# Tomeu7/AO-MARL

Measured on AMD Instinct MI355X. Metric: env steps/sec (AO frames/sec), higher is better.
Workload: dtype f32

## Files before the change

ao_marl_amd/csrc/aomarl_capi.hip:

```cpp
#include "aomarl_kernels.hip"

#include <math.h>
#include <stdlib.h>
#include <stdarg.h>
#include <stdio.h>
#include <string.h>

#include <algorithm>
#include <climits>
#include <string>
#include <vector>

static thread_local char g_err[512] = "";

int fail(const char *fmt, ...) {
  va_list ap;
  va_start(ap, fmt);
  vsnprintf(g_err, sizeof(g_err), fmt, ap);
  va_end(ap);
  return 1;
}


struct aomarl_ctx {
// ... 49 lines not shown
  bool frame_marked = false;
  struct FramePipe {
    bool have_twin = false, active = false;
    const float *owner_screens = nullptr;
    aomarl_state twin;
    int par = 0;
    hipStream_t fstream = nullptr;
    hipEvent_t ev_cmd = nullptr, ev_commit = nullptr, ev_done[2] = {nullptr, nullptr}, ev_psf[2] = {nullptr, nullptr};
    hipEvent_t ev_done_cur[2] = {nullptr, nullptr};
    bool psf_out[2] = {false, false};
    bool cmd_covers_commit = false;
    bool cmd_covers_psf = false;
    int32_t *snap[2] = {nullptr, nullptr};
    size_t snap_ints = 0;
    unsigned long long steps = 0, overlapped = 0, behind = 0;
  } pipe;
  int32_t *snap_target = nullptr;
  bool snap_complete = false;
  bool pipe_enabled = true;
  bool pipe_internal = false;
  hipEvent_t ev_frame_prev = nullptr;
  bool need_prev = false, group_overlap = false;
  bool psf_side = false;
  const float *pre_screens = nullptr;
  int pre_b = 0, pre_n = 0;
  float *cmat = nullptr;
  int ld_cmat = 0;
  int nmodes = 0, nact = 0, ld_v2m = 0, ld_m2v = 0;
  float *v2m = nullptr, *m2v = nullptr, *freedom = nullptr;
  float *s2m = nullptr;
  int s2m_nmodes = 0;
// ... 78 lines not shown

static bool is_int(float v) { return floorf(v) == v; }

int aomarl_create(const aomarl_desc *d, aomarl_ctx **out) {
  if (!d || !out) return fail("aomarl_create: null argument");
  if (d->abi_version != AOMARL_ABI_VERSION)
    return fail("aomarl_create: ABI version %d, library is %d", d->abi_version, AOMARL_ABI_VERSION);
  if (d->nlayers < 0 || d->nlayers > AOMARL_MAX_LAYERS) return fail("nlayers out of range");
  if (d->ndm < 1 || d->ndm > AOMARL_MAX_DMS) return fail("ndm out of range");
  if (d->n <= 0 || d->pupdiam <= 0 || d->n < d->pupdiam) return fail("bad pupil sizes");
  if (d->pupdiam % 4 || d->n % 4) return fail("pupil grid sizes must be multiples of 4");
  if (d->npsf & (d->npsf - 1)) return fail("npsf must be a power of two");
  if (!(d->strehl_halfwin == 4 || d->strehl_halfwin == 8 || d->strehl_halfwin == 16))
    return fail("strehl_halfwin must be 4, 8 or 16");
  aomarl_ctx *c = new aomarl_ctx();
  DevSys &s = c->sys;
  memset(&s, 0, sizeof(s));
  int rc = 0;
#define UP(T, host, n, dev)                                      \
  do {                                                           \
    T *_p;                                                       \
    rc = upload<T>(c, host, n, &_p);                             \
    if (rc) { aomarl_destroy(c); return rc; }                    \
    dev = _p;                                                    \
  } while (0)
  s.n = d->n; s.pupdiam = d->pupdiam;
  UP(float, d->mpupil, (size_t)d->n * d->n, s.mpupil);
  UP(float, d->spupil, (size_t)d->pupdiam * d->pupdiam, s.spupil);
  c->h_spupil.assign(d->spupil, d->spupil + (size_t)d->pupdiam * d->pupdiam);
  s.nvalid = d->nvalid; s.pdiam = d->pdiam; s.nfft = d->nfft; s.npix = d->npix;
// ... 397 lines not shown
  if (!c) return 0;
  for (void *p : c->owned) (void)hipFree(p);
  for (int k = 0; k < 2; k++) {
    if (c->pipe.snap[k]) (void)hipFree(c->pipe.snap[k]);
    if (c->pipe.ev_done[k]) (void)hipEventDestroy(c->pipe.ev_done[k]);
    if (c->pipe.ev_psf[k]) (void)hipEventDestroy(c->pipe.ev_psf[k]);
  }
  if (c->ev_reset) (void)hipEventDestroy(c->ev_reset);
  for (int k = 0; k < 3; k++) if (c->ev_reset2[k]) (void)hipEventDestroy(c->ev_reset2[k]);
  if (c->pipe.ev_cmd) (void)hipEventDestroy(c->pipe.ev_cmd);
  if (c->pipe.ev_commit) (void)hipEventDestroy(c->pipe.ev_commit);
  if (c->pipe.fstream) { (void)hipStreamSynchronize(c->pipe.fstream); (void)hipStreamDestroy(c->pipe.fstream); }
  if (c->atm_stream) (void)hipStreamSynchronize(c->atm_stream);
  if (c->psf_stream) (void)hipStreamSynchronize(c->psf_stream);
  if (c->ev_frame) (void)hipEventDestroy(c->ev_frame);
  if (c->ev_moved) (void)hipEventDestroy(c->ev_moved);
  if (c->ev_psf) (void)hipEventDestroy(c->ev_psf);
  if (c->env_gain) (void)hipFree(c->env_gain);
  if (c->seed_stage) (void)hipFree(c->seed_stage);
  rp_free(c);
  if (c->timg) (void)hipFree(c->timg);
  for (hipEvent_t e : c->fw_ev) (void)hipEventDestroy(e);
  for (hipEvent_t e : c->fw_ev_retired) (void)hipEventDestroy(e);
  delete c;
  return 0;
}

static int replace_dev(aomarl_ctx *c, float **slot, const std::vector<float> &h) {
  if (*slot) {
    for (size_t i = 0; i < c->owned.size(); i++)
      if (c->owned[i] == *slot) { c->owned.erase(c->owned.begin() + i); break; }
// ... 186 lines not shown
```

ao_marl_amd/csrc/aomarl_capi_atmos.hip:

```cpp
static int side_stream(aomarl_ctx *c) {
  if (!c->atm_stream) {
    int prio_lo = 0, prio_hi = 0;
    HIPCHK(hipDeviceGetStreamPriorityRange(&prio_lo, &prio_hi));
    static hipStream_t g_atm[64] = {nullptr}, g_psf[64] = {nullptr};
    int dev = 0;
    HIPCHK(hipGetDevice(&dev));
    if (dev < 0 || dev >= 64) return fail("side_stream: device ordinal %d", dev);
    if (!g_atm[dev]) {
      HIPCHK(hipStreamCreateWithPriority(&g_atm[dev], hipStreamNonBlocking, 0));
      HIPCHK(hipStreamCreateWithPriority(&g_psf[dev], hipStreamNonBlocking, prio_lo));
    }
    c->atm_stream = g_atm[dev]; c->psf_stream = g_psf[dev];
    HIPCHK(hipEventCreateWithFlags(&c->ev_frame, hipEventDisableTiming));
    c->ev_frame_cur = c->ev_frame;
    HIPCHK(hipEventCreateWithFlags(&c->ev_moved, hipEventDisableTiming));
    HIPCHK(hipEventCreateWithFlags(&c->ev_psf, hipEventDisableTiming));
    HIPCHK(hipEventCreateWithFlags(&c->ev_fork, hipEventDisableTiming));
  }
  return 0;
}
static int psf_wait_pending(aomarl_ctx *c, void *stream) {
  if (c->psf_side && !c->side_joined) HIPCHK(hipStreamWaitEvent((hipStream_t)stream, c->ev_psf, 0));
  c->psf_side = false;
  return 0;
// ... 128 lines not shown
    for (int j = 0; j < i; j++)
      if (layer[j] == layer[i]) return fail("extrude: a layer appears twice in one round");
    ops.layer[i] = layer[i]; ops.dir[i] = dir[i]; ops.tflag[i] = 0;
  }
  return extrude_rounds(c, st, b, n, &ops, 1, stream);
}

struct Plan { int kx[AOMARL_MAX_LAYERS], ky[AOMARL_MAX_LAYERS]; };

static bool plan_eq(const Plan &a, const Plan &b, int nl) {
  for (int l = 0; l < nl; l++)
    if (a.kx[l] != b.kx[l] || a.ky[l] != b.ky[l]) return false;
  return true;
}

static int run_plan(aomarl_ctx *c, aomarl_state *st, int b, int n, const Plan &p, void *stream) {
  int maxr = 0;
  for (int l = 0; l < c->nlayers; l++) {
    int len = abs(p.kx[l]) + abs(p.ky[l]);
    if (len > maxr) maxr = len;
  }
  for (int l = 0; l < c->nlayers; l++)
    if (p.kx[l] == 0 && p.ky[l] == 0) c->snap_complete = false;
  if (maxr == 0) return 0;
  if ((hipStream_t)stream != c->atm_stream || !c->atm_stream) { int rc = atmos_wait_pending(c, stream); if (rc) return rc; }
  c->group_overlap = false;
  if (c->ev_frame_prev) {
    bool fits = true;
    for (int l = 0; l < c->nlayers; l++) {
      const DevLayer &L = c->sys.layers[l];
// ... 511 lines not shown
```

ao_marl_amd/csrc/aomarl_capi_stages.hip:

```cpp
static int dm_shape_impl(aomarl_ctx *c, aomarl_state *st, int b, int n, const float *volts,
                         bool skip_stack, void *stream) {
  const float *v = volts ? volts : st->voltage + (size_t)b * st->ld_actu;
  const int ldv = volts ? c->sys.nactu : st->ld_actu;
  DevState ds = dev_state(st);
  for (int k = 0; k < c->ndm; k++) {
    const DevDm &D = c->sys.dms[k];
    const int np = D.dim * D.dim;
    if (D.type == AOMARL_DM_TT)
      hipLaunchKernelGGL(k_dm_shape, dim3(1, n), dim3(64), 0, (hipStream_t)stream, c->sys, ds, b, k, v, ldv);
    else if (skip_stack)
      continue;
    else if (D.sep && !c->force_generic_dm)
      hipLaunchKernelGGL(k_dm_shape_sep, dim3((D.dim + DMS_TX - 1) / DMS_TX, (D.dim + DMS_TY - 1) / DMS_TY, n),
                         dim3(256), 0, (hipStream_t)stream, c->sys, ds, b, k, v, ldv);
    else
      hipLaunchKernelGGL(k_dm_shape, dim3((np + 255) / 256, n), dim3(256), 0, (hipStream_t)stream, c->sys, ds, b, k, v, ldv);
    LAUNCHCHK();
  }
  return 0;
}

int aomarl_comp_dm_shape(aomarl_ctx *c, aomarl_state *st, int b, int n, const float *volts, void *stream) {
  int rc = check_range(c, st, b, n);
  if (rc) return rc;
// ... 24 lines not shown
    g_gemm_kgroups = value;
    return 0;
  }
  if (!strcmp(name, "gemm_xcd_map")) { g_gemm_xcd = value != 0; return 0; }
  if (!strcmp(name, "gemm_target_blocks")) { g_gemm_target_blocks = value > 0 ? value : 0; return 0; }
  if (!strcmp(name, "gemm_split_f16")) { g_gemm_split_f16 = value != 0; return 0; }
  if (!strcmp(name, "precision")) return aomarl_set_precision(value);
  if (!c) return fail("set_option: null context");
  if (!strcmp(name, "force_generic_dm")) { c->force_generic_dm = value != 0; return 0; }
  if (!strcmp(name, "force_valu_target")) { c->force_valu_target = value != 0; return 0; }
  if (!strcmp(name, "defer_dm_shape")) { c->defer_dm_shape = value != 0; return 0; }
  if (!strcmp(name, "frame_pipeline")) {
    if (c->pipe.active) return fail("frame_pipeline: a frame is in flight (reset first)");
    c->pipe_enabled = value != 0; return 0;
  }
  if (!strcmp(name, "small_move")) { c->small_move = value != 0; return 0; }
  if (!strcmp(name, "small_chain")) { c->small_chain = value != 0; return 0; }
  if (!strcmp(name, "renew_frame_stream")) {
    auto &P = c->pipe;
    if (P.active) return fail("renew_frame_stream: a frame is in flight (reset first)");
    if (P.fstream) {
      HIPCHK(hipStreamSynchronize(P.fstream));
      HIPCHK(hipStreamDestroy(P.fstream));
      P.fstream = nullptr;
      HIPCHK(hipStreamCreateWithFlags(&P.fstream, hipStreamNonBlocking));
    }
    return 0;
  }
  if (!strcmp(name, "residual_shortcut")) {
    if (value && (!c->s2m || c->s2m_nmodes < 1)) return fail("residual_shortcut: no v2m . cmat matrix (aomarl_set_slopes2modes)");
// ... 394 lines not shown
```

ao_marl_amd/csrc/aomarl_capi_step.hip:

```cpp
long long aomarl_actor_tiled_floats(int n_agents, int N, int K) {
  return (long long)n_agents * ((N + 15) / 16) * ((K + 15) / 16) * 256;
}

int aomarl_actor_tile_weights(int n_agents, int N, int K, const float *src, float *dst, void *stream) {
  if (!src || !dst) return fail("actor_tile_weights: null pointer");
  if (n_agents <= 0 || N <= 0 || K <= 0) return fail("actor_tile_weights: bad sizes");
  const int ntile = (N + 15) / 16, ksteps = (K + 15) / 16;
  const long long per = (long long)ntile * ksteps * 256;
  hipLaunchKernelGGL(k_actor_tile_weights, dim3((unsigned)((per + 255) / 256), n_agents), dim3(256), 0,
                     (hipStream_t)stream, N, K, ntile, ksteps, src, dst);
  LAUNCHCHK();
  return 0;
}

int aomarl_actor_forward(const aomarl_actor_desc *d, const float *state, const float *eps, uint32_t seed,
                         uint32_t counter, float *action, float *mean, void *stream) {
  if (!d || !state || !action || !mean) return fail("actor_forward: null argument");
  if (d->n_hidden < 1 || d->n_hidden > 8) return fail("actor_forward: 1..8 hidden layers");
  const int A = d->n_agents, n = d->nenv, H = d->hidden;
  if (A <= 0 || n <= 0) return 0;
  if (!(d->flags & AOMARL_ACTOR_LAYER_BY_LAYER) && d->W1_tiled && d->Whead_tiled && H % 16 == 0) {
    const int ks1 = (d->in_max + 15) / 16, nto = (2 * d->act_max + 15) / 16;
    const size_t img1 = (size_t)256 * std::max(H / 16, nto), img0 = std::max((size_t)256 * ks1, img1);
    const size_t lds = (img0 + img1 + d->act_max + 4) * sizeof(float);
// ... 96 lines not shown
      if (k < K) a0 = fmaf(xs[k], row[k], a0);
    }
    float y = a0 + a1;
    y += __shfl_xor(y, 1);
    y += __shfl_xor(y, 2);
    if (o < no && q == 0) done(o, y);
  }
}
struct SmallHead {
  int nm, na, nact, n_agents, ld_m2v, ld_actu, ktt, do_strehl;
  float gain, factor, wa, wb, wc;
  const float *m0, *m1, *action, *freedom, *m2v, *PEND;
  const int32_t *amode_inv, *lohi;
  float *modes_out, *rew;
};
__global__ __launch_bounds__(256) void k_small_head(DevSys sys, DevState st, SmallHead p) {
  __shared__ float sm[SMALL_NM], sv[SMALL_NA];
  const int e = blockIdx.x, tid = threadIdx.x, lane = tid & 63, wv = tid >> 6;
  for (int m = tid; m < p.nm; m += 256) {
    float v = p.m0[(long long)e * p.nm + m] + p.gain * p.m1[(long long)e * p.nm + m];
    if (p.action) {
      const int j = p.amode_inv[m];
      if (j >= 0) v += p.action[(long long)e * p.nact + j] * p.freedom[m];
    }
    sm[m] = v;
    if (p.modes_out) p.modes_out[(long long)e * p.nm + m] = v;
  }
  if (p.rew)
    for (int a = wv; a < p.n_agents; a += 4) {
      const int lo = p.lohi[2 * a], hi = p.lohi[2 * a + 1];
      float q = 0.f;
      for (int m = lo + lane; m < hi; m += 64) { const float v = p.m1[(long long)e * p.nm + m]; q += v * v; }
      q = wave_sum(q);
// ... 67 lines not shown
  return c->small_chain && c->sys.nactu <= SMALL_NA && c->sys.nslope <= SMALL_NSL && g->nmodes <= SMALL_NM &&
         (long long)c->sys.nactu * c->sys.nslope <= 65536 && c->cmat && !c->env_gain;
}

static bool env_step_fusable(aomarl_ctx *c, const aomarl_env_glue *g, int *ktt_out) {
  int ktt = -1, ntt = 0, nother = 0;
  for (int k = 0; k < c->ndm; k++) {
    if (c->sys.dms[k].type == AOMARL_DM_TT) { ktt = k; ntt++; } else nother++;
  }
  const bool defer = c->defer_dm_shape && aomarl_dm_from_voltage_available(c);
  if (ktt_out) *ktt_out = ktt;
  return !(g->flags & AOMARL_ENV_STEP_UNFUSED) && ntt == 1 && (defer || nother == 0);
}

static int env_step_head_fused(aomarl_ctx *c, aomarl_state *st, aomarl_state *stv, aomarl_env_glue *g, const float *action,
                               float gain, float *reward_out, int ktt, bool ahead, hipEvent_t psf_ev, void *stream) {
  hipStream_t s = (hipStream_t)stream;
  const int n = st->nenv, nm = g->nmodes, R = g->nhist + 1, na = c->sys.nactu;
  const size_t slot = (size_t)n * nm;
  float *newest = g->modes_ring + (size_t)g->ring_pos * slot;
  float *mnew = g->modes_ring + (size_t)((g->ring_pos + 1) % R) * slot;
  Work w = work_layout(c, st->nenv);
  DevState dsv = dev_state(stv);
  if (small_chain_ok(c, g)) {
    const float d = c->delay;
    SmallHead p;
    if (d <= 1.f) { p.wa = 1.f - d; p.wb = d; p.wc = 0.f; } else { p.wa = 0.f; p.wb = 2.f - d; p.wc = d - 1.f; }
    if (ahead) { p.wa = p.wb; p.wb = p.wc; p.wc = 0.f; }
    p.nm = nm; p.na = na; p.nact = c->nact; p.n_agents = reward_out ? g->n_agents : 0; p.ld_m2v = c->ld_m2v;
    p.ld_actu = st->ld_actu; p.ktt = ktt; p.do_strehl = 1; p.gain = gain; p.factor = g->reward_factor;
    p.m0 = newest; p.m1 = g->res_modes; p.action = action; p.freedom = c->freedom; p.m2v = c->m2v;
    p.PEND = stv->work + w.PEND; p.amode_inv = c->amode_inv; p.lohi = g->lohi; p.modes_out = mnew; p.rew = reward_out;
    if (psf_ev) HIPCHK(hipStreamWaitEvent(s, psf_ev, 0));
    else if (stv == st) { int rc = psf_wait_pending(c, stream); if (rc) return rc; }
    hipExtLaunchKernelGGL(k_small_head, dim3(n), dim3(256), 0, s, nullptr, ahead ? c->pipe.ev_cmd : nullptr, 0, c->sys, dsv, p);
    LAUNCHCHK();
    if (ahead) c->pipe.cmd_covers_commit = true;
    return 0;
  }
  float *modes = st->work + w.MODES;
  const int cx = (nm + 255) / 256;
  bool psf_waited = false;
  if (ahead && psf_ev) { HIPCHK(hipStreamWaitEvent(s, psf_ev, 0)); psf_waited = true; }
  hipLaunchKernelGGL(k_compose_rewards, dim3(cx + (reward_out ? g->n_agents : 0), n), dim3(256), 0, s, nm, newest,
                     g->res_modes, gain, action, c->nact, c->amode_inv, c->freedom, modes, w.ldm, mnew, cx,
                     g->n_agents, g->lohi, g->reward_factor, reward_out);
  LAUNCHCHK();
  int nsp = 0;
  float alpha = 1.f;
  launch_gemm_nt(n, na, nm, 1.0f, modes, w.ldm, c->m2v, c->ld_m2v, 0.0f, st->com, st->ld_actu, s,
                 st->work + w.GEMM, w.gemm_floats, nullptr, &nsp, true, 16.f, c->m2v_scale, &alpha, 288);
  LAUNCHCHK();
  const float d = c->delay;
  float wa, wb, wc;
  if (d <= 1.f) { wa = 1.f - d; wb = d; wc = 0.f; } else { wa = 0.f; wb = 2.f - d; wc = d - 1.f; }
  if (ahead) {
    hipExtLaunchKernelGGL(k_delay_ahead, dim3((na + 255) / 256, 2 * n), dim3(256), 0, s, nullptr, c->pipe.ev_cmd, 0, c->sys, dsv, na,
                          st->ld_actu, n, nsp > 0 ? st->work + w.GEMM : nullptr, nsp, alpha, ktt);
    LAUNCHCHK();
    c->pipe.cmd_covers_psf = psf_waited;
  } else {
    if (nsp > 0)
      hipLaunchKernelGGL(k_delay_sum, dim3((na + 255) / 256, n), dim3(256), 0, s, dsv, na, st->ld_actu, wa, wb, wc, 0, 1,
                         st->work + w.GEMM, nsp, alpha, n);
    else
      hipLaunchKernelGGL(k_delay, dim3((na + 255) / 256, n), dim3(256), 0, s, dsv, na, st->ld_actu, wa, wb, wc, 0, 1);
    LAUNCHCHK();
  }
  if (psf_ev) { if (!psf_waited) HIPCHK(hipStreamWaitEvent(s, psf_ev, 0)); }
  else if (stv == st) { int rc = psf_wait_pending(c, stream); if (rc) return rc; }
  hipLaunchKernelGGL(k_post_delay, dim3(ahead ? n : 2 * n), dim3(256), 0, s, c->sys, dsv, 0, n, stv->work + w.PEND, 1, ktt,
                     stv->voltage, st->ld_actu);
  LAUNCHCHK();
// ... 154 lines not shown
  const auto &P = c->pipe;
  return P.have_twin && c->pipe_enabled && P.owner_screens == st->screens && !c->graph_step && !c->capturing && c->prefetch_atmos &&
         c->delay == 1.f && c->sys.noise < 0.f && !g->denoiser && accumx && accumy && !c->subpixel_flow &&
         aomarl_frame_fused_available(c) && c->defer_dm_shape && aomarl_dm_from_voltage_available(c) &&
         env_step_fusable(c, g, nullptr);
}

static int pipe_init(aomarl_ctx *c, const aomarl_state *st) {
  auto &P = c->pipe;
  int rc = side_stream(c);
  if (rc) return rc;
  if (!P.fstream) {
    HIPCHK(hipStreamCreateWithFlags(&P.fstream, hipStreamNonBlocking));
    HIPCHK(hipEventCreateWithFlags(&P.ev_cmd, hipEventDisableTiming));
    HIPCHK(hipEventCreateWithFlags(&P.ev_commit, hipEventDisableTiming));
    for (int k = 0; k < 2; k++) {
      HIPCHK(hipEventCreateWithFlags(&P.ev_done[k], hipEventDisableTiming));
      HIPCHK(hipEventCreateWithFlags(&P.ev_psf[k], hipEventDisableTiming));
    }
  }
  const size_t ints = (size_t)st->nenv * c->nlayers * 2;
  if (P.snap_ints < ints) {
    for (int k = 0; k < 2; k++) {
      if (P.snap[k]) (void)hipFree(P.snap[k]);
      P.snap[k] = nullptr;
      HIPCHK(hipMalloc((void **)&P.snap[k], sizeof(int32_t) * ints));
    }
    P.snap_ints = ints;
  }
  return 0;
}

static int pipe_launch_frame(aomarl_ctx *c, aomarl_state *st, int q, void *stream) {
  auto &P = c->pipe;
  (void)stream;
  HIPCHK(hipStreamWaitEvent(P.fstream, P.ev_cmd, 0));
  if (!c->premoved || c->pre_screens != st->screens || c->pre_b != 0 || c->pre_n != st->nenv)
    return fail("frame pipeline: no prefetched atmosphere frame of the whole batch is pending");
  HIPCHK(hipStreamWaitEvent(P.fstream, c->ev_moved, 0));
  c->premoved = false;
  aomarl_state v = pipe_view(c, st, q);
  v.origin = P.snap[q];
  return frame_fused_impl(c, &v, 0, st->nenv, AOMARL_IMG_COG | AOMARL_IMG_NOISE | AOMARL_IMG_DM_FROM_VOLTAGE,
                          (void *)P.fstream, q);
}

static int pipe_prefetch(aomarl_ctx *c, aomarl_state *st, float *accumx, float *accumy, int older, int newest) {
  auto &P = c->pipe;
  if (c->premoved) return fail("frame pipeline: a prefetched frame is already pending");
  c->side_joined = false;
  c->ev_frame_prev = P.ev_done_cur[older]; c->need_prev = true;
  c->ev_frame_cur = P.ev_done_cur[newest]; c->frame_wait_pending = true;
  c->snap_target = P.snap[older]; c->snap_complete = true;
  c->ride_ev = c->ev_moved; c->rode = false;
  int rc = move_atmos_now(c, st, 0, st->nenv, accumx, accumy, (void *)c->atm_stream);
  c->ride_ev = nullptr;
  const bool complete = c->snap_complete;
  c->snap_target = nullptr;
  if (!rc && !complete && c->need_prev && c->frame_wait_pending)
    rc = hipStreamWaitEvent(c->atm_stream, c->ev_frame_prev, 0) == hipSuccess ? 0 : fail("frame pipeline: hipStreamWaitEvent failed");
  c->ev_frame_prev = nullptr; c->need_prev = false; c->frame_wait_pending = false; c->group_overlap = false;
  if (rc) return rc;
  if (!complete)
    HIPCHK(hipMemcpyAsync(P.snap[older], st->origin, sizeof(int32_t) * (size_t)st->nenv * c->nlayers * 2,
                          hipMemcpyDeviceToDevice, c->atm_stream));
  c->screens_dirty_main = false;
  if (!(c->rode && complete)) HIPCHK(hipEventRecord(c->ev_moved, c->atm_stream));
  c->premoved = true; c->pre_screens = st->screens; c->pre_b = 0; c->pre_n = st->nenv;
  return 0;
}

static int env_step_pipelined(aomarl_ctx *c, aomarl_state *st, aomarl_env_glue *g, const float *action, float gain,
                              float *accumx, float *accumy, float *state_out, float *reward_out, void *stream) {
// ... 12 lines not shown
    HIPCHK(hipEventRecord(P.ev_psf[0], c->psf_stream));
    P.psf_out[0] = true; P.psf_out[1] = false;
    c->psf_side = false;
    aomarl_state v1 = pipe_view(c, st, 1);
    HIPCHK(hipMemcpyAsync(v1.voltage, st->com1, sizeof(float) * (size_t)n * st->ld_actu, hipMemcpyDeviceToDevice, s));
    Work w = work_layout(c, st->nenv);
    hipLaunchKernelGGL(k_post_delay, dim3(2 * n), dim3(256), 0, s, c->sys, dev_state(&v1), 0, n, v1.work + w.PEND, 0, ktt,
                       v1.voltage, st->ld_actu);
    LAUNCHCHK();
    HIPCHK(hipEventRecord(P.ev_cmd, s));
    HIPCHK(hipEventRecord(P.ev_commit, s));
    P.cmd_covers_commit = false;
    HIPCHK(hipMemcpyAsync(P.snap[1], st->origin, sizeof(int32_t) * (size_t)n * c->nlayers * 2, hipMemcpyDeviceToDevice,
                          c->atm_stream));
    HIPCHK(hipEventRecord(c->ev_moved, c->atm_stream));
    c->pipe_internal = true;
    rc = pipe_launch_frame(c, st, 1, stream);
    if (!rc) rc = pipe_prefetch(c, st, accumx, accumy, 0, 1);
    c->pipe_internal = false;
    if (rc) return rc;
    P.active = true; P.par = 1;
    return 0;
  }
  const int p = P.par, q = 1 - p;
  c->pipe_internal = true;
  int rc = env_step_validate(c, st, g, action, state_out, reward_out);
  aomarl_state vq = pipe_view(c, st, q), vp = pipe_view(c, st, p);
  hipEvent_t pe = P.psf_out[q] ? P.ev_psf[q] : nullptr;
  if (!rc) rc = env_step_head_fused(c, st, &vq, g, action, gain, reward_out, ktt, true, pe, stream);
  if (!rc && pe && !P.cmd_covers_commit && !P.cmd_covers_psf && hipStreamWaitEvent(P.fstream, pe, 0) != hipSuccess) rc = fail("frame pipeline: hipStreamWaitEvent failed");
  if (!rc) { P.psf_out[q] = false; P.cmd_covers_psf = false; rc = pipe_launch_frame(c, st, q, stream); }
  if (!rc) rc = pipe_prefetch(c, st, accumx, accumy, p, q);
  if (!rc && hipStreamWaitEvent(s, P.ev_done_cur[p], 0) != hipSuccess) rc = fail("frame pipeline: hipStreamWaitEvent failed");
  if (!rc && small_chain_ok(c, g)) rc = env_step_tail(c, st, g, true, state_out, stream, &vp);
  else if (!rc && env_step_shortcut(c, g)) rc = env_step_tail(c, st, g, true, state_out, stream, nullptr, &vp);
  else {
    if (!rc) rc = aomarl_do_control(c, &vp, 0, n, stream);
    if (!rc) rc = env_step_tail(c, st, g, true, state_out, stream);
  }
  c->pipe_internal = false;
  if (rc) return rc;
  P.par = q; P.steps++;
  return 0;
}

static int pipe_drop(aomarl_ctx *c, void *stream) {
  auto &P = c->pipe;
  hipStream_t s = (hipStream_t)stream;
  if (P.ev_done_cur[P.par]) HIPCHK(hipStreamWaitEvent(s, P.ev_done_cur[P.par], 0));
  for (int k = 0; k < 2; k++)
    if (P.psf_out[k]) { HIPCHK(hipStreamWaitEvent(s, P.ev_psf[k], 0)); P.psf_out[k] = false; }
  P.active = false; P.par = 0;
  return 0;
}

int aomarl_set_frame_pipeline(aomarl_ctx *c, const aomarl_state *st, const aomarl_state *twin) {
  if (!c) return fail("set_frame_pipeline: null context");
  auto &P = c->pipe;
  if (P.active) return fail("set_frame_pipeline: a frame is in flight (reset first)");
  if (!twin) { P.have_twin = false; P.owner_screens = nullptr; return 0; }
  if (!st) return fail("set_frame_pipeline: null state");
  int rc = check_range(c, st, 0, st->nenv);
  if (rc) return rc;
  if (twin->nenv != st->nenv || twin->ld_actu != st->ld_actu) return fail("set_frame_pipeline: the twin's nenv / ld_actu differ");
  if (twin->screens != st->screens || twin->origin != st->origin || twin->seeds != st->seeds || twin->ext_count != st->ext_count ||
      twin->com != st->com || twin->com1 != st->com1 || twin->com2 != st->com2 || twin->err != st->err ||
      twin->strehl != st->strehl || twin->le_img != st->le_img || twin->frame != st->frame)
// ... 25 lines not shown
      if (e == 0) { p.kx[l] = kx; p.ky[l] = ky; }
      else if (p.kx[l] != kx || p.ky[l] != ky) return false;
    }
  return true;
}

int aomarl_policy_env_step(aomarl_ctx *c, aomarl_state *st, aomarl_env_glue *g, const aomarl_actor_desc *d,
                           const float *state, const float *eps, uint32_t seed, uint32_t counter, float gain,
                           float *accumx, float *accumy, float *action, float *mean, float *state_out,
                           float *reward_out, void *stream) {
  if (!c || !st || !g || !d || !state || !action || !mean || !state_out) return fail("policy_env_step: null argument");
  if (d->nenv != st->nenv) return fail("policy_env_step: the actors are set up for %d environments, the state has %d", d->nenv, st->nenv);
  int rc = aomarl_actor_forward(d, state, eps, seed, counter, action, mean, stream);
  if (rc) return rc;
  return aomarl_env_step(c, st, g, action, gain, accumx, accumy, state_out, reward_out, stream);
}

int aomarl_do_control_reduced(aomarl_ctx *c, aomarl_state *st, void *stream) {
  if (!c || !st) return fail("do_control_reduced: null argument");
  auto &P = c->pipe;
  if (!(P.active && P.owner_screens == st->screens)) return aomarl_do_control(c, st, 0, st->nenv, stream);
  aomarl_state v = pipe_view(c, st, 1 - P.par);
  c->pipe_internal = true;
  const int rc = aomarl_do_control(c, &v, 0, st->nenv, stream);
  c->pipe_internal = false;
  return rc;
}

int aomarl_env_step_shortcut(aomarl_ctx *c, const aomarl_env_glue *g) {
  if (!c || !g) return 0;
// ... 145 lines not shown
```

ao_marl_amd/csrc/aomarl_dev.h:

```cpp
#pragma once
#include <hip/hip_runtime.h>
#include <hip/hip_ext.h>
#include <stdint.h>

#include "../../include/aomarl.h"

#ifndef CHAIN_PRIO
#define CHAIN_PRIO 0
#endif
#define CHAIN_SETPRIO() do { if (CHAIN_PRIO) __builtin_amdgcn_s_setprio(CHAIN_PRIO); } while (0)
#ifndef ATM_PRIO
#define ATM_PRIO 0
#endif
#define ATM_SETPRIO() do { if (ATM_PRIO) __builtin_amdgcn_s_setprio(ATM_PRIO); } while (0)
typedef float f32x4 __attribute__((ext_vector_type(4)));
typedef float f32x16 __attribute__((ext_vector_type(16)));
typedef _Float16 hx2 __attribute__((ext_vector_type(2)));
typedef _Float16 hx8 __attribute__((ext_vector_type(8)));
__device__ __forceinline__ f32x4 mfma_h(hx8 a, hx8 b, f32x4 c) {
  return __builtin_amdgcn_mfma_f32_16x16x32_f16(a, b, c, 0, 0, 0);
}

struct DevLayer {
  int dim, ns;
// ... 62 lines not shown
  const float *tt_pk;
};

struct DevState {
  int nenv, ld_actu;
  float *screens;
  int32_t *origin;
  uint32_t *seeds, *ext_count;
  float *com, *com1, *com2, *err, *voltage, *slopes, *dm_shape, *bincube, *wfs_phase, *tar_phase;
  float *strehl, *le_img;
  uint32_t *frame;
  float *work;
  int32_t *origin_snap;
};

template <int B, typename F>
__device__ __forceinline__ float slab_sum(int nsplit, F at) {
  float acc = 0.f;
  for (int z0 = 0; z0 < nsplit; z0 += B) {
    float pz[B];
#pragma unroll
    for (int z = 0; z < B; z++) pz[z] = at(min(z0 + z, nsplit - 1));
#pragma unroll
    for (int z = 0; z < B; z++) acc = (z0 + z < nsplit) ? acc + pz[z] : acc;
  }
  return acc;
}

__device__ __forceinline__ void philox4x32_10(uint32_t c0, uint32_t c1, uint32_t c2, uint32_t c3,
                                              uint32_t k0, uint32_t k1, uint32_t out[4]) {
// ... 92 lines not shown
```

ao_marl_amd/csrc/aomarl_kernels.hip:

```cpp
#include "aomarl_host.h"
#include "aomarl_gemm_p.h"
#include <type_traits>

#define WAVE 64

typedef unsigned u32x4 __attribute__((ext_vector_type(4)));

__device__ __forceinline__ hx2 cvt_h2(float a, float b) {
  return __builtin_bit_cast(hx2, __builtin_amdgcn_cvt_pkrtz(a, b));
}
__device__ __forceinline__ float sub_lo(hx2 h, float a) {
  float r;
  asm("v_fma_mix_f32 %0, %1, -1.0, %2 op_sel_hi:[1,0,0]" : "=v"(r) : "v"(h), "v"(a));
  return r;
}
__device__ __forceinline__ float sub_hi(hx2 h, float a) {
  float r;
  asm("v_fma_mix_f32 %0, %1, -1.0, %2 op_sel:[1,0,0] op_sel_hi:[1,0,0]" : "=v"(r) : "v"(h), "v"(a));
  return r;
}

struct __attribute__((packed, aligned(4))) f4u { float v[4]; };
__device__ __forceinline__ void add4(float acc[4], const float *p) {
  const f4u t = *reinterpret_cast<const f4u *>(p);
// ... 2631 lines not shown
  const long long o = (long long)e * ld + i;
  const float s = slab_sum<4>(nsplit, [&](int z) { return P[((long long)z * nrows + blockIdx.y) * nactu + i]; });
  const float c0 = alpha * s;
  st.com[o] = c0;
  if (comp_voltage) {
    const float c1 = st.com1[o], c2 = st.com2[o];
    st.voltage[o] = a * c0 + b * c1 + c * c2;
    st.com2[o] = c1;
    st.com1[o] = c0;
  } else {
    st.voltage[o] = c0;
  }
}

__global__ void k_delay_ahead(DevSys sys, DevState st, int nactu, int ld, int n, const float *__restrict__ P,
                              int nsplit, float alpha, int ktt) {
  CHAIN_SETPRIO();
  auto newest = [&](int row, int a) -> float {
    if (nsplit > 0) {
      return alpha * slab_sum<4>(nsplit, [&](int z) { return P[((long long)z * n + row) * nactu + a]; });
    }
    return st.com[(long long)row * ld + a];
  };
  if ((int)blockIdx.y < n) {
    const int e = blockIdx.y, i = blockIdx.x * blockDim.x + threadIdx.x;
    if (i >= nactu) return;
    const long long o = (long long)e * ld + i;
    const float c0 = newest(e, i);
    if (nsplit > 0) st.com[o] = c0;
    const float c1 = st.com1[o];
    st.voltage[o] = c0;
    st.com2[o] = c1;
    st.com1[o] = c0;
  } else if (blockIdx.x == 0 && ktt >= 0) {
    const int row = blockIdx.y - n, p = threadIdx.x;
    const DevDm &D = sys.dms[ktt];
    float *shape = st.dm_shape + (long long)row * sys.shape_stride + D.shape_off;
    if (p < 2) shape[p] = newest(row, D.com_off + p);
    if (p == 2 && sys.fused_ok) {
      const DevDm &Z = sys.dms[0];
      const int half = sys.pupdiam / 2, zp = (half + Z.toy) * Z.dim + half + Z.tox;
      const int ss2 = Z.ss * Z.ss, s0 = Z.influstart[zp], cn = Z.ninflu[zp];
      float acc = 0.f;
      for (int t = 0; t < cn; t++) {
        const int pos = Z.influpos[s0 + t];
        acc += Z.influ[pos] * newest(row, Z.com_off + pos / ss2);
      }
      shape[2] = acc;
    }
  }
// ... 656 lines not shown
```

ao_marl_amd/libaomarl.py:

```python
import ctypes as C
import os
import subprocess

import numpy as np

HERE = os.path.dirname(os.path.abspath(__file__))
LIB_PATH = os.environ.get("AOMARL_LIB") or os.path.join(HERE, "libaomarl_hip.so")
MAX_LAYERS, MAX_DMS, ABI_VERSION = 8, 4, 2
PRECISION_F32, PRECISION_SPLIT_F16 = 0, 1

DM_PZT, DM_TT = 0, 1
TRACE_ATMOS, TRACE_DMS, TRACE_RESET, TRACE_MASK = 1, 2, 4, 8
IMG_FROM_PHASE_BUFFER, IMG_NOISE, IMG_WRITE_BINCUBE, IMG_COG, IMG_NO_ATMOS, IMG_NO_DMS = \
    1, 2, 4, 8, 16, 32
IMG_DM_FROM_VOLTAGE = 64
APPLY_COMP_VOLTAGE, APPLY_DEFER_STACK_SHAPE = 1, 2

_fp = C.POINTER(C.c_float)
_ip = C.POINTER(C.c_int32)
_up = C.POINTER(C.c_uint32)


class DmDesc(C.Structure):
    _fields_ = [("type", C.c_int32), ("dim", C.c_int32), ("nact", C.c_int32),
# ... 102 lines not shown
    ("aomarl_assemble_state_cols", _i, [_i, _i, C.POINTER(C.c_void_p), _ip, _ip, C.POINTER(C.c_void_p),
                                        C.POINTER(C.c_void_p), _vp, _vp, _vp]),
    ("aomarl_agent_rewards", _i, [_i, _i, _i, _vp, _i, _vp, C.c_float, _vp, _vp]),
    ("aomarl_actor_tiled_floats", C.c_longlong, [_i, _i, _i]),
    ("aomarl_actor_tile_weights", _i, [_i, _i, _i, _vp, _vp, _vp]),
    ("aomarl_actor_forward", _i, [_vp, _vp, _vp, C.c_uint32, C.c_uint32, _vp, _vp, _vp]),
    ("aomarl_env_step", _i, [_vp, C.POINTER(State), _vp, _vp, _f, _fp, _fp, _vp, _vp, _vp]),
    ("aomarl_policy_env_step", _i, [_vp, C.POINTER(State), _vp, _vp, _vp, _vp, C.c_uint32, C.c_uint32, _f, _fp, _fp,
                                    _vp, _vp, _vp, _vp, _vp]),
    ("aomarl_env_step_shortcut", _i, [_vp, _vp]),
    ("aomarl_do_control_reduced", _i, [_vp, C.POINTER(State), _vp]),
    ("aomarl_graph_stats", _i, [_vp, C.POINTER(C.c_ulonglong), C.POINTER(C.c_ulonglong)]),
    ("aomarl_set_frame_pipeline", _i, [_vp, C.POINTER(State), C.POINTER(State)]),
    ("aomarl_frame_pipeline_state", _i, [_vp, C.POINTER(_i), C.POINTER(_i), C.POINTER(C.c_ulonglong),
                                         C.POINTER(C.c_ulonglong)]),
    ("aomarl_frame_kernel_name", C.c_char_p, [_vp]),
    ("aomarl_frame_kernel_time", _i, [_vp, C.POINTER(C.c_double), C.POINTER(_i)]),
    ("aomarl_denoiser_create", _i, [C.POINTER(_fp), C.POINTER(_fp), C.POINTER(C.c_void_p)]),
    ("aomarl_denoiser_apply", _i, [_vp, _vp, C.c_longlong, _vp]),
    ("aomarl_denoiser_apply_f32", _i, [_vp, _vp, C.c_longlong, _vp]),
    ("aomarl_denoiser_apply_split_f16", _i, [_vp, _vp, C.c_longlong, _vp]),
    ("aomarl_denoiser_overflow", _i, [_vp, C.POINTER(C.c_uint), _vp]),
    ("aomarl_denoiser_destroy", _i, [_vp]),
    ("aomarl_target_psf_buffer", _i, _range + [_vp]),
    ("aomarl_set_geo", _i, [_vp, _fp]),
    ("aomarl_geo_workspace_floats", C.c_size_t, [_vp, _i]),
    ("aomarl_geo_control", _i, _range + [_vp, _vp]),
    ("aomarl_frame_fused_available", _i, [_vp]),
    ("aomarl_dm_from_voltage_available", _i, [_vp]),
    ("aomarl_materialize_dm_shape", _i, _range + [_vp]),
# ... 340 lines not shown
```

ao_marl_amd/sim.py:

```python
import ctypes as C

import numpy as np
import torch

from . import libaomarl as la
from . import system


def _ld4(n):
    return (n + 3) & ~3


def hip_calibration_id():
    import os
    st = os.stat(la.LIB_PATH)
    return ("hip", os.path.abspath(la.LIB_PATH), int(st.st_size), int(st.st_mtime_ns), str(la.get_precision()))


class HipSim(object):
    def __init__(self, s, nenv, device="cuda:0", keep_bincube=False, keep_phase=False):
        if not torch.cuda.is_available():
            raise la.AomarlError("HipSim needs a GPU (torch.cuda.is_available() is False); the "
                                 "product path has no CPU fallback")
        self.lib = la.load()
# ... 109 lines not shown
              "work": torch.zeros(self.t["work"].numel(), **f32)}
        st2 = la.State()
        for name, _ in la.State._fields_:
            setattr(st2, name, getattr(self.st, name))
        for k, v in tw.items():
            setattr(st2, k, v.data_ptr())
        la.check(self.lib.aomarl_set_frame_pipeline(self.ctx, C.byref(self.st), C.byref(st2)))
        self._twin, self._twin_st = tw, st2

    def frame_pipeline_state(self):
        a, b = C.c_int(0), C.c_int(0)
        n, o = C.c_ulonglong(0), C.c_ulonglong(0)
        la.check(self.lib.aomarl_frame_pipeline_state(self.ctx, C.byref(a), C.byref(b), C.byref(n), C.byref(o)))
        return bool(a.value), bool(b.value), int(n.value), int(o.value)

    def _frame_buf(self, name):
        if getattr(self, "_twin", None) is not None and self.frame_pipeline_state()[1]:
            return self._twin[name]
        return self.t[name]

    @property
    def strehl(self):
        s = self.t["strehl"]
        avg = torch.where(s[:, 4] > 0, s[:, 3] / s[:, 4].clamp(min=1), torch.zeros_like(s[:, 3]))
        return torch.stack([s[:, 0], s[:, 1], s[:, 2], avg], dim=1)

    @property
    def strehl_fit(self):
        la.check(self.lib.aomarl_strehl_fit(self.ctx, C.byref(self.st), 0, self.nenv, self._stream()))
        s = self.t["strehl"]
# ... 641 lines not shown
```

include/aomarl.h:

```cpp
#ifndef AOMARL_H
#define AOMARL_H
#include <stddef.h>
#include <stdint.h>

#ifdef __cplusplus
extern "C" {
#endif

#define AOMARL_MAX_LAYERS 8
#define AOMARL_MAX_DMS 4
#define AOMARL_ABI_VERSION 2

enum { AOMARL_DM_PZT = 0, AOMARL_DM_TT = 1 };

enum { AOMARL_TRACE_ATMOS = 1, AOMARL_TRACE_DMS = 2, AOMARL_TRACE_RESET = 4,
       AOMARL_TRACE_MASK = 8  };
enum {
  AOMARL_IMG_FROM_PHASE_BUFFER = 1,
  AOMARL_IMG_NOISE = 2,
  AOMARL_IMG_WRITE_BINCUBE = 4,
  AOMARL_IMG_COG = 8,
  AOMARL_IMG_NO_ATMOS = 16,
  AOMARL_IMG_NO_DMS = 32,
  AOMARL_IMG_DM_FROM_VOLTAGE = 64
// ... 234 lines not shown
#define AOMARL_ENV_STEP_UNFUSED 1
int aomarl_env_step(aomarl_ctx *ctx, aomarl_state *st, aomarl_env_glue *glue, const float *action_dev,
                    float gain, float *accumx, float *accumy, float *state_out, float *reward_out,
                    void *stream);
int aomarl_policy_env_step(aomarl_ctx *ctx, aomarl_state *st, aomarl_env_glue *glue, const aomarl_actor_desc *d,
                           const float *state_dev, const float *eps_dev, uint32_t seed, uint32_t counter, float gain,
                           float *accumx, float *accumy, float *action_dev, float *mean_dev, float *state_out,
                           float *reward_out, void *stream);
int aomarl_env_step_shortcut(aomarl_ctx *ctx, const aomarl_env_glue *glue);
int aomarl_do_control_reduced(aomarl_ctx *ctx, aomarl_state *st, void *stream);
int aomarl_graph_stats(aomarl_ctx *ctx, unsigned long long *captures, unsigned long long *replays);

int aomarl_set_frame_pipeline(aomarl_ctx *ctx, const aomarl_state *st, const aomarl_state *twin);
int aomarl_frame_pipeline_state(aomarl_ctx *ctx, int *in_flight, int *consumed_in_twin,
                                unsigned long long *steps, unsigned long long *overlapped);

typedef struct aomarl_denoiser aomarl_denoiser;
int aomarl_denoiser_create(const float *const *weights, const float *const *biases,
                           aomarl_denoiser **out);
int aomarl_denoiser_apply(aomarl_denoiser *dn, float *cube, long long nimg, void *stream);
int aomarl_denoiser_apply_f32(aomarl_denoiser *dn, float *cube, long long nimg, void *stream);
int aomarl_denoiser_apply_split_f16(aomarl_denoiser *dn, float *cube, long long nimg, void *stream);
int aomarl_denoiser_overflow(aomarl_denoiser *dn, unsigned *count, void *stream);
int aomarl_denoiser_destroy(aomarl_denoiser *dn);
int aomarl_target_psf_buffer(aomarl_ctx *ctx, aomarl_state *st, int env_begin, int env_count,
                             void *stream);
int aomarl_target_image(aomarl_ctx *ctx, aomarl_state *st, int env_begin, int env_count, float *out, void *stream);
int aomarl_set_geo(aomarl_ctx *ctx, const float *W);
size_t aomarl_geo_workspace_floats(aomarl_ctx *ctx, int nenv);
int aomarl_geo_control(aomarl_ctx *ctx, aomarl_state *st, int env_begin, int env_count,
// ... 34 lines not shown
```

Baseline: 542,100.

## Compute next frame's screen origins in head kernel so frame launch skips atmosphere move

When the host can predict the next atmosphere shift as a few uniform groups, the per-env screen origins for the next frame are computed directly inside the fused head kernel (k_small_head / k_delay_ahead) from the previous snapshot. The frame kernel can then wait on the previous move event rather than the current one, so it no longer waits for the current atmosphere move to finish. This adds double-buffered move events, a pending-plan record and epoch checks, plus a diagnostic API. The risk is subtle ordering bugs between the atmosphere and frame streams and the snapshot buffers.

```diff
diff --git a/ao_marl_amd/csrc/aomarl_capi.hip b/ao_marl_amd/csrc/aomarl_capi.hip
--- a/ao_marl_amd/csrc/aomarl_capi.hip
+++ b/ao_marl_amd/csrc/aomarl_capi.hip
@@ -87,7 +87,19 @@
     int32_t *snap[2] = {nullptr, nullptr};
     size_t snap_ints = 0;
     unsigned long long steps = 0, overlapped = 0, behind = 0;
+    hipEvent_t ev_mv[2] = {nullptr, nullptr};
+    int mv_cur = 0;
+    hipEvent_t snap_ev[2] = {nullptr, nullptr};
+    int head_read = -1;
+    struct Pending {
+      bool valid = false;
+      int ng = 0, end[SNAP_GROUPS];
+      int16_t kx[SNAP_GROUPS][AOMARL_MAX_LAYERS], ky[SNAP_GROUPS][AOMARL_MAX_LAYERS];
+      unsigned long long epoch = 0, gepoch = 0;
+    } pend;
+    unsigned long long ahead = 0;
   } pipe;
+  bool frame_ahead = true;
   int32_t *snap_target = nullptr;
   bool snap_complete = false;
   bool pipe_enabled = true;
@@ -196,6 +208,7 @@
   if (!(d->strehl_halfwin == 4 || d->strehl_halfwin == 8 || d->strehl_halfwin == 16))
     return fail("strehl_halfwin must be 4, 8 or 16");
   aomarl_ctx *c = new aomarl_ctx();
+  { const char *e = getenv("AOMARL_FRAME_AHEAD"); if (e && atol(e) == 0) c->frame_ahead = false; }
   DevSys &s = c->sys;
   memset(&s, 0, sizeof(s));
   int rc = 0;
@@ -623,7 +636,8 @@
   if (c->atm_stream) (void)hipStreamSynchronize(c->atm_stream);
   if (c->psf_stream) (void)hipStreamSynchronize(c->psf_stream);
   if (c->ev_frame) (void)hipEventDestroy(c->ev_frame);
-  if (c->ev_moved) (void)hipEventDestroy(c->ev_moved);
+  if (c->pipe.ev_mv[0]) { for (int k = 0; k < 2; k++) (void)hipEventDestroy(c->pipe.ev_mv[k]); }
+  else if (c->ev_moved) (void)hipEventDestroy(c->ev_moved);
   if (c->ev_psf) (void)hipEventDestroy(c->ev_psf);
   if (c->env_gain) (void)hipFree(c->env_gain);
   if (c->seed_stage) (void)hipFree(c->seed_stage);
diff --git a/ao_marl_amd/csrc/aomarl_capi_atmos.hip b/ao_marl_amd/csrc/aomarl_capi_atmos.hip
--- a/ao_marl_amd/csrc/aomarl_capi_atmos.hip
+++ b/ao_marl_amd/csrc/aomarl_capi_atmos.hip
@@ -166,6 +166,40 @@
   return true;
 }
 
+static bool plan_fits_incoming(const aomarl_ctx *c, const Plan &p) {
+  for (int l = 0; l < c->nlayers; l++) {
+    const DevLayer &L = c->sys.layers[l];
+    const int lox = L.tox, hix = L.dim - L.tox - c->sys.pupdiam, loy = L.toy, hiy = L.dim - L.toy - c->sys.pupdiam;
+    if ((p.kx[l] > 0 ? p.kx[l] > hix : -p.kx[l] > lox) || (p.ky[l] > 0 ? p.ky[l] > hiy : -p.ky[l] > loy)) return false;
+  }
+  return true;
+}
+
+static bool pipe_plan_ahead(aomarl_ctx *c, int n, const float *accumx, const float *accumy) {
+  auto &Q = c->pipe.pend;
+  const int nl = c->nlayers;
+  Q.ng = 0;
+  Plan cur;
+  for (int e = 0; e <= n; e++) {
+    Plan p;
+    if (e < n)
+      for (int l = 0; l < nl; l++) {
+        p.kx[l] = (int)(accumx[(size_t)e * nl + l] + c->deltax[l]);
+        p.ky[l] = (int)(accumy[(size_t)e * nl + l] + c->deltay[l]);
+      }
+    if (e == 0) { cur = p; continue; }
+    if (e == n || !plan_eq(p, cur, nl)) {
+      if (Q.ng == SNAP_GROUPS || !plan_fits_incoming(c, cur)) return false;
+      for (int l = 0; l < AOMARL_MAX_LAYERS; l++) {
+        Q.kx[Q.ng][l] = l < nl ? (int16_t)cur.kx[l] : 0; Q.ky[Q.ng][l] = l < nl ? (int16_t)cur.ky[l] : 0;
+      }
+      Q.end[Q.ng++] = e;
+      cur = p;
+    }
+  }
+  return Q.ng > 0;
+}
+
 static int run_plan(aomarl_ctx *c, aomarl_state *st, int b, int n, const Plan &p, void *stream) {
   int maxr = 0;
   for (int l = 0; l < c->nlayers; l++) {
diff --git a/ao_marl_amd/csrc/aomarl_capi_stages.hip b/ao_marl_amd/csrc/aomarl_capi_stages.hip
--- a/ao_marl_amd/csrc/aomarl_capi_stages.hip
+++ b/ao_marl_amd/csrc/aomarl_capi_stages.hip
@@ -62,6 +62,7 @@
     if (c->pipe.active) return fail("frame_pipeline: a frame is in flight (reset first)");
     c->pipe_enabled = value != 0; return 0;
   }
+  if (!strcmp(name, "frame_ahead_of_move")) { c->frame_ahead = value != 0; return 0; }
   if (!strcmp(name, "small_move")) { c->small_move = value != 0; return 0; }
   if (!strcmp(name, "small_chain")) { c->small_chain = value != 0; return 0; }
   if (!strcmp(name, "renew_frame_stream")) {
diff --git a/ao_marl_amd/csrc/aomarl_capi_step.hip b/ao_marl_amd/csrc/aomarl_capi_step.hip
--- a/ao_marl_amd/csrc/aomarl_capi_step.hip
+++ b/ao_marl_amd/csrc/aomarl_capi_step.hip
@@ -134,9 +134,10 @@
   const int32_t *amode_inv, *lohi;
   float *modes_out, *rew;
 };
-__global__ __launch_bounds__(256) void k_small_head(DevSys sys, DevState st, SmallHead p) {
+__global__ __launch_bounds__(256) void k_small_head(DevSys sys, DevState st, SmallHead p, SnapAhead sa) {
   __shared__ float sm[SMALL_NM], sv[SMALL_NA];
   const int e = blockIdx.x, tid = threadIdx.x, lane = tid & 63, wv = tid >> 6;
+  if (sa.dst && tid >= 192 && tid - 192 < sys.nlayers) snap_ahead_entry(sys, sa, e, tid - 192);
   for (int m = tid; m < p.nm; m += 256) {
     float v = p.m0[(long long)e * p.nm + m] + p.gain * p.m1[(long long)e * p.nm + m];
     if (p.action) {
@@ -234,7 +235,10 @@
 }
 
 static int env_step_head_fused(aomarl_ctx *c, aomarl_state *st, aomarl_state *stv, aomarl_env_glue *g, const float *action,
-                               float gain, float *reward_out, int ktt, bool ahead, hipEvent_t psf_ev, void *stream) {
+                               float gain, float *reward_out, int ktt, bool ahead, hipEvent_t psf_ev, void *stream,
+                               const SnapAhead *sa = nullptr) {
+  SnapAhead sa0;
+  if (ahead && sa) sa0 = *sa; else { memset(&sa0, 0, sizeof(sa0)); sa0.dst = nullptr; }
   hipStream_t s = (hipStream_t)stream;
   const int n = st->nenv, nm = g->nmodes, R = g->nhist + 1, na = c->sys.nactu;
   const size_t slot = (size_t)n * nm;
@@ -253,7 +257,7 @@
     p.PEND = stv->work + w.PEND; p.amode_inv = c->amode_inv; p.lohi = g->lohi; p.modes_out = mnew; p.rew = reward_out;
     if (psf_ev) HIPCHK(hipStreamWaitEvent(s, psf_ev, 0));
     else if (stv == st) { int rc = psf_wait_pending(c, stream); if (rc) return rc; }
-    hipExtLaunchKernelGGL(k_small_head, dim3(n), dim3(256), 0, s, nullptr, ahead ? c->pipe.ev_cmd : nullptr, 0, c->sys, dsv, p);
+    hipExtLaunchKernelGGL(k_small_head, dim3(n), dim3(256), 0, s, nullptr, ahead ? c->pipe.ev_cmd : nullptr, 0, c->sys, dsv, p, sa0);
     LAUNCHCHK();
     if (ahead) c->pipe.cmd_covers_commit = true;
     return 0;
@@ -276,7 +280,7 @@
   if (d <= 1.f) { wa = 1.f - d; wb = d; wc = 0.f; } else { wa = 0.f; wb = 2.f - d; wc = d - 1.f; }
   if (ahead) {
     hipExtLaunchKernelGGL(k_delay_ahead, dim3((na + 255) / 256, 2 * n), dim3(256), 0, s, nullptr, c->pipe.ev_cmd, 0, c->sys, dsv, na,
-                          st->ld_actu, n, nsp > 0 ? st->work + w.GEMM : nullptr, nsp, alpha, ktt);
+                          st->ld_actu, n, nsp > 0 ? st->work + w.GEMM : nullptr, nsp, alpha, ktt, sa0);
     LAUNCHCHK();
     c->pipe.cmd_covers_psf = psf_waited;
   } else {
@@ -461,6 +465,8 @@
     HIPCHK(hipStreamCreateWithFlags(&P.fstream, hipStreamNonBlocking));
     HIPCHK(hipEventCreateWithFlags(&P.ev_cmd, hipEventDisableTiming));
     HIPCHK(hipEventCreateWithFlags(&P.ev_commit, hipEventDisableTiming));
+    P.ev_mv[0] = c->ev_moved; P.mv_cur = 0;
+    HIPCHK(hipEventCreateWithFlags(&P.ev_mv[1], hipEventDisableTiming));
     for (int k = 0; k < 2; k++) {
       HIPCHK(hipEventCreateWithFlags(&P.ev_done[k], hipEventDisableTiming));
       HIPCHK(hipEventCreateWithFlags(&P.ev_psf[k], hipEventDisableTiming));
@@ -478,13 +484,26 @@
   return 0;
 }
 
-static int pipe_launch_frame(aomarl_ctx *c, aomarl_state *st, int q, void *stream) {
+static int pipe_launch_frame(aomarl_ctx *c, aomarl_state *st, int q, void *stream, bool ahead = false) {
   auto &P = c->pipe;
   (void)stream;
   HIPCHK(hipStreamWaitEvent(P.fstream, P.ev_cmd, 0));
   if (!c->premoved || c->pre_screens != st->screens || c->pre_b != 0 || c->pre_n != st->nenv)
     return fail("frame pipeline: no prefetched atmosphere frame of the whole batch is pending");
-  HIPCHK(hipStreamWaitEvent(P.fstream, c->ev_moved, 0));
+  if (ahead) {
+    HIPCHK(hipStreamWaitEvent(P.fstream, P.ev_mv[P.mv_cur ^ 1], 0));
+    P.ahead++;
+  } else {
+    if (P.pend.valid) {
+      if (P.ev_done_cur[q]) HIPCHK(hipStreamWaitEvent(c->atm_stream, P.ev_done_cur[q], 0));
+      HIPCHK(hipMemcpyAsync(P.snap[q], st->origin, sizeof(int32_t) * (size_t)st->nenv * c->nlayers * 2, hipMemcpyDeviceToDevice,
+                            c->atm_stream));
+      HIPCHK(hipEventRecord(c->ev_moved, c->atm_stream));
+      P.snap_ev[q] = c->ev_moved;
+    }
+    HIPCHK(hipStreamWaitEvent(P.fstream, c->ev_moved, 0));
+  }
+  P.pend.valid = false;
   c->premoved = false;
   aomarl_state v = pipe_view(c, st, q);
   v.origin = P.snap[q];
@@ -498,12 +517,18 @@
   c->side_joined = false;
   c->ev_frame_prev = P.ev_done_cur[older]; c->need_prev = true;
   c->ev_frame_cur = P.ev_done_cur[newest]; c->frame_wait_pending = true;
-  c->snap_target = P.snap[older]; c->snap_complete = true;
+  P.mv_cur ^= 1; c->ev_moved = P.ev_mv[P.mv_cur];
+  const bool ahead = c->frame_ahead && pipe_plan_ahead(c, st->nenv, accumx, accumy);
+  P.pend.valid = ahead; P.pend.epoch = c->cfg_epoch; P.pend.gepoch = g_cfg_epoch;
+  if (!ahead && P.head_read == older)
+    HIPCHK(hipStreamWaitEvent(c->atm_stream, P.ev_cmd, 0));
+  c->snap_target = ahead ? nullptr : P.snap[older]; c->snap_complete = true;
   c->ride_ev = c->ev_moved; c->rode = false;
   int rc = move_atmos_now(c, st, 0, st->nenv, accumx, accumy, (void *)c->atm_stream);
   c->ride_ev = nullptr;
-  const bool complete = c->snap_complete;
+  const bool complete = ahead || c->snap_complete;
   c->snap_target = nullptr;
+  if (!ahead) P.snap_ev[older] = c->ev_moved;
   if (!rc && !complete && c->need_prev && c->frame_wait_pending)
     rc = hipStreamWaitEvent(c->atm_stream, c->ev_frame_prev, 0) == hipSuccess ? 0 : fail("frame pipeline: hipStreamWaitEvent failed");
   c->ev_frame_prev = nullptr; c->need_prev = false; c->frame_wait_pending = false; c->group_overlap = false;
@@ -546,6 +571,7 @@
     HIPCHK(hipMemcpyAsync(P.snap[1], st->origin, sizeof(int32_t) * (size_t)n * c->nlayers * 2, hipMemcpyDeviceToDevice,
                           c->atm_stream));
     HIPCHK(hipEventRecord(c->ev_moved, c->atm_stream));
+    P.snap_ev[1] = c->ev_moved; P.snap_ev[0] = nullptr; P.pend.valid = false; P.head_read = -1;
     c->pipe_internal = true;
     rc = pipe_launch_frame(c, st, 1, stream);
     if (!rc) rc = pipe_prefetch(c, st, accumx, accumy, 0, 1);
@@ -559,9 +585,20 @@
   int rc = env_step_validate(c, st, g, action, state_out, reward_out);
   aomarl_state vq = pipe_view(c, st, q), vp = pipe_view(c, st, p);
   hipEvent_t pe = P.psf_out[q] ? P.ev_psf[q] : nullptr;
-  if (!rc) rc = env_step_head_fused(c, st, &vq, g, action, gain, reward_out, ktt, true, pe, stream);
+  SnapAhead sa;
+  memset(&sa, 0, sizeof(sa));
+  const bool fa = !rc && P.pend.valid && c->frame_ahead && P.pend.epoch == c->cfg_epoch && P.pend.gepoch == g_cfg_epoch;
+  P.head_read = -1;
+  if (fa) {
+    sa.dst = P.snap[q]; sa.src = P.snap[p]; sa.ng = P.pend.ng;
+    for (int k = 0; k < SNAP_GROUPS; k++) sa.end[k] = k < sa.ng ? P.pend.end[k] : n;
+    memcpy(sa.kx, P.pend.kx, sizeof(sa.kx)); memcpy(sa.ky, P.pend.ky, sizeof(sa.ky));
+    if (P.snap_ev[p] && hipStreamWaitEvent(s, P.snap_ev[p], 0) != hipSuccess) rc = fail("frame pipeline: hipStreamWaitEvent failed");
+    P.snap_ev[p] = nullptr; P.snap_ev[q] = nullptr; P.head_read = p;
+  }
+  if (!rc) rc = env_step_head_fused(c, st, &vq, g, action, gain, reward_out, ktt, true, pe, stream, fa ? &sa : nullptr);
   if (!rc && pe && !P.cmd_covers_commit && !P.cmd_covers_psf && hipStreamWaitEvent(P.fstream, pe, 0) != hipSuccess) rc = fail("frame pipeline: hipStreamWaitEvent failed");
-  if (!rc) { P.psf_out[q] = false; P.cmd_covers_psf = false; rc = pipe_launch_frame(c, st, q, stream); }
+  if (!rc) { P.psf_out[q] = false; P.cmd_covers_psf = false; rc = pipe_launch_frame(c, st, q, stream, fa); }
   if (!rc) rc = pipe_prefetch(c, st, accumx, accumy, p, q);
   if (!rc && hipStreamWaitEvent(s, P.ev_done_cur[p], 0) != hipSuccess) rc = fail("frame pipeline: hipStreamWaitEvent failed");
   if (!rc && small_chain_ok(c, g)) rc = env_step_tail(c, st, g, true, state_out, stream, &vp);
@@ -583,6 +620,7 @@
   for (int k = 0; k < 2; k++)
     if (P.psf_out[k]) { HIPCHK(hipStreamWaitEvent(s, P.ev_psf[k], 0)); P.psf_out[k] = false; }
   P.active = false; P.par = 0;
+  P.pend.valid = false; P.head_read = -1; P.snap_ev[0] = P.snap_ev[1] = nullptr;
   return 0;
 }
 
@@ -638,6 +676,18 @@
   int rc = aomarl_actor_forward(d, state, eps, seed, counter, action, mean, stream);
   if (rc) return rc;
   return aomarl_env_step(c, st, g, action, gain, accumx, accumy, state_out, reward_out, stream);
+}
+
+int aomarl_frame_pipeline_ahead(aomarl_ctx *c, unsigned long long *ahead, int32_t *origins, int count) {
+  if (!c) return fail("frame_pipeline_ahead: null context");
+  if (ahead) *ahead = c->pipe.ahead;
+  if (origins) {
+    const auto &P = c->pipe;
+    if (!P.active || count < 0 || (size_t)count > P.snap_ints) return fail("frame_pipeline_ahead: no frame in flight, or count beyond nenv * nlayers * 2");
+    HIPCHK(hipDeviceSynchronize());
+    HIPCHK(hipMemcpy(origins, P.snap[P.par], sizeof(int32_t) * (size_t)count, hipMemcpyDeviceToHost));
+  }
+  return 0;
 }
 
 int aomarl_do_control_reduced(aomarl_ctx *c, aomarl_state *st, void *stream) {
diff --git a/ao_marl_amd/csrc/aomarl_dev.h b/ao_marl_amd/csrc/aomarl_dev.h
--- a/ao_marl_amd/csrc/aomarl_dev.h
+++ b/ao_marl_amd/csrc/aomarl_dev.h
@@ -100,6 +100,24 @@
   int32_t *origin_snap;
 };
 
+constexpr int SNAP_GROUPS = 4;
+struct SnapAhead {
+  int32_t *dst;
+  const int32_t *src;
+  int ng, end[SNAP_GROUPS];
+  int16_t kx[SNAP_GROUPS][AOMARL_MAX_LAYERS], ky[SNAP_GROUPS][AOMARL_MAX_LAYERS];
+};
+__device__ __forceinline__ void snap_ahead_entry(const DevSys &sys, const SnapAhead &sa, int e, int l) {
+  int g = 0;
+#pragma unroll
+  for (int k = 1; k < SNAP_GROUPS; k++) if (k < sa.ng && e >= sa.end[k - 1]) g = k;
+  const int n = sys.layers[l].dim, i = (e * sys.nlayers + l) * 2;
+  int x = sa.src[i] + sa.kx[g][l], y = sa.src[i + 1] + sa.ky[g][l];
+  x -= (x >= n) ? n : 0; x += (x < 0) ? n : 0;
+  y -= (y >= n) ? n : 0; y += (y < 0) ? n : 0;
+  sa.dst[i] = x; sa.dst[i + 1] = y;
+}
+
 template <int B, typename F>
 __device__ __forceinline__ float slab_sum(int nsplit, F at) {
   float acc = 0.f;
diff --git a/ao_marl_amd/csrc/aomarl_kernels.hip b/ao_marl_amd/csrc/aomarl_kernels.hip
--- a/ao_marl_amd/csrc/aomarl_kernels.hip
+++ b/ao_marl_amd/csrc/aomarl_kernels.hip
@@ -2669,7 +2669,7 @@
 }
 
 __global__ void k_delay_ahead(DevSys sys, DevState st, int nactu, int ld, int n, const float *__restrict__ P,
-                              int nsplit, float alpha, int ktt) {
+                              int nsplit, float alpha, int ktt, SnapAhead sa) {
   CHAIN_SETPRIO();
   auto newest = [&](int row, int a) -> float {
     if (nsplit > 0) {
@@ -2687,8 +2687,10 @@
     st.voltage[o] = c0;
     st.com2[o] = c1;
     st.com1[o] = c0;
-  } else if (blockIdx.x == 0 && ktt >= 0) {
+  } else if (blockIdx.x == 0) {
     const int row = blockIdx.y - n, p = threadIdx.x;
+    if (sa.dst && p >= 64 && p - 64 < sys.nlayers) snap_ahead_entry(sys, sa, row, p - 64);
+    if (ktt < 0) return;
     const DevDm &D = sys.dms[ktt];
     float *shape = st.dm_shape + (long long)row * sys.shape_stride + D.shape_off;
     if (p < 2) shape[p] = newest(row, D.com_off + p);
diff --git a/ao_marl_amd/libaomarl.py b/ao_marl_amd/libaomarl.py
--- a/ao_marl_amd/libaomarl.py
+++ b/ao_marl_amd/libaomarl.py
@@ -140,6 +140,7 @@
     ("aomarl_set_frame_pipeline", _i, [_vp, C.POINTER(State), C.POINTER(State)]),
     ("aomarl_frame_pipeline_state", _i, [_vp, C.POINTER(_i), C.POINTER(_i), C.POINTER(C.c_ulonglong),
                                          C.POINTER(C.c_ulonglong)]),
+    ("aomarl_frame_pipeline_ahead", _i, [_vp, C.POINTER(C.c_ulonglong), _vp, _i]),
     ("aomarl_frame_kernel_name", C.c_char_p, [_vp]),
     ("aomarl_frame_kernel_time", _i, [_vp, C.POINTER(C.c_double), C.POINTER(_i)]),
     ("aomarl_denoiser_create", _i, [C.POINTER(_fp), C.POINTER(_fp), C.POINTER(C.c_void_p)]),
diff --git a/ao_marl_amd/sim.py b/ao_marl_amd/sim.py
--- a/ao_marl_amd/sim.py
+++ b/ao_marl_amd/sim.py
@@ -147,6 +147,15 @@
         la.check(self.lib.aomarl_frame_pipeline_state(self.ctx, C.byref(a), C.byref(b), C.byref(n), C.byref(o)))
         return bool(a.value), bool(b.value), int(n.value), int(o.value)
 
+    def frame_pipeline_ahead(self, origins=False):
+        a = C.c_ulonglong(0)
+        if not origins:
+            la.check(self.lib.aomarl_frame_pipeline_ahead(self.ctx, C.byref(a), None, 0))
+            return int(a.value)
+        o = np.zeros((self.nenv, max(self.s.nscreens, 1), 2), dtype=np.int32)
+        la.check(self.lib.aomarl_frame_pipeline_ahead(self.ctx, C.byref(a), o.ctypes.data_as(C.c_void_p), o.size))
+        return int(a.value), o
+
     def _frame_buf(self, name):
         if getattr(self, "_twin", None) is not None and self.frame_pipeline_state()[1]:
             return self._twin[name]
diff --git a/include/aomarl.h b/include/aomarl.h
--- a/include/aomarl.h
+++ b/include/aomarl.h
@@ -272,6 +272,7 @@
 int aomarl_set_frame_pipeline(aomarl_ctx *ctx, const aomarl_state *st, const aomarl_state *twin);
 int aomarl_frame_pipeline_state(aomarl_ctx *ctx, int *in_flight, int *consumed_in_twin,
                                 unsigned long long *steps, unsigned long long *overlapped);
+int aomarl_frame_pipeline_ahead(aomarl_ctx *ctx, unsigned long long *ahead, int32_t *origins, int count);
 
 typedef struct aomarl_denoiser aomarl_denoiser;
 int aomarl_denoiser_create(const float *const *weights, const float *const *biases,
```

Result: no change. 542,000 (median of 2 runs) (-0.0%).
